# nianlonggu/WhisperSeg

Hardware: AMD Instinct MI355X
Metric: audio-sec/s segmented (whisperseg-large, 30 s windows) (higher is better)
Workload: dtype f16x3

## Files before the change

### whisperseg_amd/csrc/wseg_enc.hip

```cpp
#include <stdlib.h>
#include <string.h>
#include "wseg_kernels.h"

namespace wseg {

template <typename T>
__global__ __launch_bounds__(256) void im2col_conv1_kernel(const float* __restrict__ x, void* __restrict__ a1,
                                                           int C, int cols, int kp) {
  constexpr int TT = 32;
  __shared__ float tile[96][TT + 2 + 1];
  const int b = blockIdx.y, t0 = blockIdx.x * TT;
  for (int i = threadIdx.x; i < C * (TT + 2); i += 256) {
    const int c = i / (TT + 2), j = i - c * (TT + 2);
    const int t = t0 + j - 1;
    tile[c][j] = (t >= 0 && t < cols) ? x[((size_t)b * C + c) * cols + t] : 0.f;
  }
  __syncthreads();
  for (int i = threadIdx.x; i < TT * kp; i += 256) {
    const int tt = i / kp, k = i - tt * kp;
    if (t0 + tt >= cols) continue;
    float v = 0.f;
    if (k < 3 * C) {
      const int tap = k / C, c = k - tap * C;
      v = tile[c][tt + tap];
    }
    Op<T>::st1(a1, (size_t)b * cols + t0 + tt, kp, k, v);
  }
}

template <typename T>
__global__ __launch_bounds__(256) void im2col_conv2_kernel(const T* __restrict__ h1, T* __restrict__ a2,
                                                           int B, int cols, int d) {
  constexpr int V = 16 / sizeof(T);
  const int dv = d / V, half = cols / 2;
  const size_t total = (size_t)B * half * 3 * dv;
  for (size_t i = (size_t)blockIdx.x * 256 + threadIdx.x; i < total; i += (size_t)gridDim.x * 256) {
    const int cv = (int)(i % dv);
    const size_t r = i / dv;
    const int tap = (int)(r % 3);
    const size_t bt = r / 3;
    const int t = (int)(bt % half), b = (int)(bt / half);
    const int src = 2 * t + tap - 1;
    uint4 v = make_uint4(0, 0, 0, 0);
    if (src >= 0 && src < cols) v = *(const uint4*)(h1 + ((size_t)b * cols + src) * d + (size_t)cv * V);
    *(uint4*)(a2 + (bt * 3 + tap) * d + (size_t)cv * V) = v;
  }
}

template <typename T> struct VecIO {
  static __device__ __forceinline__ void ld(const T* p, float v[8]) { unpack8<T>(*(const uint4*)p, v); }
  static __device__ __forceinline__ void st(T* p, const float v[8]) { *(uint4*)p = pack8<T>(v); }
};
template <> struct VecIO<float> {
  static __device__ __forceinline__ void ld(const float* p, float v[8]) {
    const float4 a = *(const float4*)p, b = *(const float4*)(p + 4);
    v[0] = a.x; v[1] = a.y; v[2] = a.z; v[3] = a.w; v[4] = b.x; v[5] = b.y; v[6] = b.z; v[7] = b.w;
  }
  static __device__ __forceinline__ void st(float* p, const float v[8]) {
    *(float4*)p = make_float4(v[0], v[1], v[2], v[3]);
    *(float4*)(p + 4) = make_float4(v[4], v[5], v[6], v[7]);
  }
};

template <typename TO, int NIT>
__global__ __launch_bounds__(256) void layernorm_kernel(const float* __restrict__ x, const typename IO<TO>::P* __restrict__ g,
                                                        const typename IO<TO>::P* __restrict__ bta, void* __restrict__ y, int M, int d) {
  typedef typename IO<TO>::P PT;
  constexpr int V = 8;
  const int row = blockIdx.x * 4 + (threadIdx.x >> 6), lane = threadIdx.x & 63;
  if (row >= M) return;
  const float* xr = x + (size_t)row * d;
  float v[NIT][V];
  float sum = 0.f;
#pragma unroll
  for (int it = 0; it < NIT; ++it) {
    const int c = (it * 64 + lane) * V;
    if (c < d) {
      VecIO<float>::ld(xr + c, v[it]);
#pragma unroll
      for (int j = 0; j < V; ++j) sum += v[it][j];
    } else {
#pragma unroll
      for (int j = 0; j < V; ++j) v[it][j] = 0.f;
    }
  }
  const float mean = wave_sum(sum) / (float)d;
  float sq = 0.f;
#pragma unroll
  for (int it = 0; it < NIT; ++it) {
    const int c = (it * 64 + lane) * V;
    if (c < d) {
#pragma unroll
      for (int j = 0; j < V; ++j) { const float t = v[it][j] - mean; sq += t * t; }
    }
  }
  const float rstd = 1.0f / sqrtf(wave_sum(sq) / (float)d + 1e-5f);
#pragma unroll
  for (int it = 0; it < NIT; ++it) {
    const int c = (it * 64 + lane) * V;
    if (c < d) {
      float gg[V], bb[V], o[V];
      VecIO<PT>::ld(g + c, gg);
      VecIO<PT>::ld(bta + c, bb);
#pragma unroll
      for (int j = 0; j < V; ++j) o[j] = (v[it][j] - mean) * rstd * gg[j] + bb[j];
      op_st8<TO>(y, (size_t)row, d, c, o);
    }
  }
}

template <typename HT, typename TO, bool SPLIT = false>
__global__ __launch_bounds__(256, SPLIT ? 3 : 4) void enc_attention_h16_kernel(const HT* __restrict__ Q, const HT* __restrict__ K,
                                                                const HT* __restrict__ Vt, void* __restrict__ out,
                                                                 int H, int T, int Tp, int d, size_t plane) {
  __shared__ __attribute__((aligned(16))) HT sK[2][64 * 64];
  __shared__ __attribute__((aligned(16))) HT sV[64 * 64];
  __shared__ __attribute__((aligned(16))) HT sKl[SPLIT ? 2 : 1][SPLIT ? 64 * 64 : 8];
  __shared__ __attribute__((aligned(16))) HT sVl[SPLIT ? 64 * 64 : 8];
  const int tid = threadIdx.x, lane = tid & 63;
  const int wave = __builtin_amdgcn_readfirstlane(tid >> 6);
  const int bh = blockIdx.y, b = bh / H, h = bh - b * H;
  const int q0 = blockIdx.x * 128 + wave * 32;
  const int qi = lane & 31, g2 = lane >> 5;
  const HT* Qb = Q + enc_qk_index(bh, Tp, 0);
  const HT* Kb = K + enc_qk_index(bh, Tp, 0);
  const HT* Vb = Vt + enc_vt_block(bh, Tp);

  bf16x8 qf[4], qfl[SPLIT ? 4 : 1];
#pragma unroll
  for (int hs = 0; hs < 4; ++hs) qf[hs] = *(const bf16x8*)(Qb + (size_t)(q0 + qi) * 64 + hs * 16 + g2 * 8);
  if constexpr (SPLIT) {
#pragma unroll
    for (int hs = 0; hs < 4; ++hs) qfl[hs] = *(const bf16x8*)(Qb + plane + (size_t)(q0 + qi) * 64 + hs * 16 + g2 * 8);
  }

  f32x16 o0, o1;
#pragma unroll
  for (int r = 0; r < 16; ++r) { o0[r] = 0.f; o1[r] = 0.f; }
  float m_run = -1.0e30f, l_run = 0.f;

  const int n_tiles = (T + 63) / 64;
  const unsigned kfrag = (unsigned)(qi * 128 + ((g2 ^ ((qi >> 1) & 7)) << 4));
  constexpr int NDMA = SPLIT ? 4 : 2;
  auto fetch_tile = [&](const HT* src, HT* dst, HT* dst_lo) {
#pragma unroll
    for (int i = 0; i < 2; ++i) {
      const int c = tid + i * 256, row = c >> 3, sl = (c & 7) ^ ((row >> 1) & 7);
      __builtin_amdgcn_global_load_lds((const __attribute__((address_space(1))) void*)(src + row * 64 + sl * 8),
                                       (__attribute__((address_space(3))) void*)(dst + (i * 256 + wave * 64) * 8), 16, 0, 0);
      if constexpr (SPLIT)
        __builtin_amdgcn_global_load_lds((const __attribute__((address_space(1))) void*)(src + plane + row * 64 + sl * 8),
                                         (__attribute__((address_space(3))) void*)(dst_lo + (i * 256 + wave * 64) * 8), 16, 0, 0);
    }
  };
  auto fetch_k = [&](int kt) { fetch_tile(Kb + (size_t)(kt * 64) * 64, sK[kt & 1], sKl[kt & 1]); };
  auto fetch_v = [&](int kt) { fetch_tile(Vb + (size_t)kt * 64 * 64, sV, sVl); };
  fetch_k(0);
  for (int kt = 0; kt < n_tiles; ++kt) {
    const HT* cK = sK[kt & 1];
    asm volatile("s_waitcnt vmcnt(0)" ::: "memory");
    __syncthreads();
    fetch_v(kt);
    const bool more = kt + 1 < n_tiles;
    if (more) fetch_k(kt + 1);
    {
      const int key_base = kt * 64;
      f32x16 s0, s1;
#pragma unroll
      for (int r = 0; r < 16; ++r) { s0[r] = 0.f; s1[r] = 0.f; }
      unsigned kfo = kfrag;
      asm volatile("" : "+v"(kfo));
      const char* cKs = (const char*)cK;
      [[maybe_unused]] const char* cKls = (const char*)sKl[kt & 1];
      __builtin_amdgcn_s_setprio(1);
#pragma unroll
      for (int hs = 0; hs < 4; ++hs) {
        const bf16x8 kf0 = *(const bf16x8*)(cKs + (kfo ^ (hs << 5)));
        const bf16x8 kf1 = *(const bf16x8*)(cKs + 4096 + (kfo ^ (hs << 5)));
        s0 = H16<HT>::mfma32(kf0, qf[hs], s0);
        s1 = H16<HT>::mfma32(kf1, qf[hs], s1);
        if constexpr (SPLIT) {
          const bf16x8 kfl0 = *(const bf16x8*)(cKls + (kfo ^ (hs << 5)));
          const bf16x8 kfl1 = *(const bf16x8*)(cKls + 4096 + (kfo ^ (hs << 5)));
          s0 = H16<HT>::mfma32(kf0, qfl[hs], s0);
          s1 = H16<HT>::mfma32(kf1, qfl[hs], s1);
          s0 = H16<HT>::mfma32(kfl0, qf[hs], s0);
          s1 = H16<HT>::mfma32(kfl1, qf[hs], s1);
        }
      }
      __builtin_amdgcn_s_setprio(0);
      if (key_base + 64 > T) {
        asm volatile("");
#pragma unroll
        for (int r = 0; r < 16; ++r) {
          const int key = key_base + (r & 3) + 8 * (r >> 2) + 4 * g2;
          if (key >= T) s0[r] = -1.0e30f;
          if (key + 32 >= T) s1[r] = -1.0e30f;
        }
      }
      float mx = fmaxf(s0[0], s1[0]);
#pragma unroll
      for (int r = 1; r < 16; ++r) mx = fmaxf(fmaxf(mx, s0[r]), s1[r]);
      mx = fmaxf(mx, lane_xor<32>(mx));
      const float m_new = fmaxf(m_run, mx);
      const float alpha = __expf(m_run - m_new);
      float ps = 0.f;
      const float m_l2 = -m_new * 1.4426950408889634f;
#pragma unroll
      for (int r = 0; r < 16; ++r) {
        s0[r] = __builtin_amdgcn_exp2f(fmaf(s0[r], 1.4426950408889634f, m_l2));
        s1[r] = __builtin_amdgcn_exp2f(fmaf(s1[r], 1.4426950408889634f, m_l2));
        ps += s0[r] + s1[r];
      }
      m_run = m_new;
      if (__builtin_amdgcn_ballot_w64(alpha != 1.0f)) {
#pragma unroll
        for (int r = 0; r < 16; ++r) { o0[r] *= alpha; o1[r] *= alpha; }
      }
      if (more) asm volatile("s_waitcnt vmcnt(%0) lgkmcnt(0)" ::"n"(NDMA) : "memory");
      else asm volatile("s_waitcnt vmcnt(0) lgkmcnt(0)" ::: "memory");
      __builtin_amdgcn_s_barrier();
      asm volatile("" ::: "memory");
      __builtin_amdgcn_s_setprio(1);
#pragma unroll
      for (int sub = 0; sub < 2; ++sub) {
        const f32x16& sv = sub == 0 ? s0 : s1;
#pragma unroll
        for (int mm = 0; mm < 2; ++mm) {
          union { bf16x8 v; uint32_t u[4]; } pf, pfl;
#pragma unroll
          for (int jj = 0; jj < 4; ++jj) pf.u[jj] = H16<HT>::pack(sv[8 * mm + 2 * jj], sv[8 * mm + 2 * jj + 1]);
          if constexpr (SPLIT) {
#pragma unroll
            for (int jj = 0; jj < 4; ++jj)
              pfl.u[jj] = H16<HT>::pack(H16<HT>::sub_lo(sv[8 * mm + 2 * jj], pf.u[jj]), H16<HT>::sub_hi(sv[8 * mm + 2 * jj + 1], pf.u[jj]));
          }
#pragma unroll
          for (int ht = 0; ht < 2; ++ht) {
            const bf16x8 vf = *(const bf16x8*)((const char*)sV + ht * 4096 + (kfo ^ ((sub * 2 + mm) << 5)));
            if (ht == 0) o0 = H16<HT>::mfma32(vf, pf.v, o0);
            else o1 = H16<HT>::mfma32(vf, pf.v, o1);
            if constexpr (SPLIT) {
              const bf16x8 vfl = *(const bf16x8*)((const char*)sVl + ht * 4096 + (kfo ^ ((sub * 2 + mm) << 5)));
              if (ht == 0) { o0 = H16<HT>::mfma32(vf, pfl.v, o0); o0 = H16<HT>::mfma32(vfl, pf.v, o0); }
              else { o1 = H16<HT>::mfma32(vf, pfl.v, o1); o1 = H16<HT>::mfma32(vfl, pf.v, o1); }
            }
          }
        }
      }
      __builtin_amdgcn_s_setprio(0);
      ps += lane_xor<32>(ps);
      l_run = l_run * alpha + ps;
    }
  }
  const int q = q0 + qi;
  if constexpr (IsMx<TO>::v) {
    const float inv = 1.0f / l_run;
    uint32_t hw[2][8], lw[2][8];
    float amax_h[2] = {0.f, 0.f}, amax_l[2] = {0.f, 0.f};
#pragma unroll
    for (int ht = 0; ht < 2; ++ht) {
      const f32x16& o = ht == 0 ? o0 : o1;
#pragma unroll
      for (int p = 0; p < 8; ++p) {
        const float a0 = H16<f16_t>::sat(o[2 * p] * inv), a1 = H16<f16_t>::sat(o[2 * p + 1] * inv);
        const uint32_t hh = H16<f16_t>::pack(a0, a1);
        const float r0 = a0 - H16<f16_t>::lo(hh), r1 = a1 - H16<f16_t>::hi(hh);
        const uint32_t ll = H16<f16_t>::pack(r0, r1);
        hw[ht][p] = hh; lw[ht][p] = ll;
        amax_h[ht] = fmaxf(amax_h[ht], fmaxf(fabsf(H16<f16_t>::lo(hh)), fabsf(H16<f16_t>::hi(hh))));
        amax_l[ht] = fmaxf(amax_l[ht], fmaxf(fabsf(H16<f16_t>::lo(ll)), fabsf(H16<f16_t>::hi(ll))));
      }
    }
    uint32_t gh[16], gl[16];
    float ah = g2 ? amax_h[1] : amax_h[0], al = g2 ? amax_l[1] : amax_l[0];
    ah = fmaxf(ah, lane_xor<32>(g2 ? amax_h[0] : amax_h[1]));
    al = fmaxf(al, lane_xor<32>(g2 ? amax_l[0] : amax_l[1]));
#pragma unroll
    for (int p = 0; p < 8; ++p) {
      const uint32_t mine_h = g2 ? hw[1][p] : hw[0][p], give_h = g2 ? hw[0][p] : hw[1][p];
      const uint32_t mine_l = g2 ? lw[1][p] : lw[0][p], give_l = g2 ? lw[0][p] : lw[1][p];
      const uint32_t got_h = lane_xor_u<32>(give_h), got_l = lane_xor_u<32>(give_l);
      const int rg = p >> 1, pr = p & 1;
      gh[4 * rg + pr] = g2 ? got_h : mine_h;
      gh[4 * rg + 2 + pr] = g2 ? mine_h : got_h;
      gl[4 * rg + pr] = g2 ? got_l : mine_l;
      gl[4 * rg + 2 + pr] = g2 ? mine_l : got_l;
    }
    if (q < T) {
      const size_t row = (size_t)b * T + q;
      const int c = h * 64 + g2 * 32;
      unsigned char* blk = (unsigned char*)out + row * (size_t)(4 * d) + (size_t)(c >> 6) * 256;
#pragma unroll
      for (int i = 0; i < 4; ++i) *(uint4*)(blk + (c & 63) * 2 + 16 * i) = make_uint4(gh[4 * i], gh[4 * i + 1], gh[4 * i + 2], gh[4 * i + 3]);
      uint4 c0, c1;
      const int chunk = (c >> 5) & 1;
      mx_chunk(gl, al, c0, c1);
      *(uint4*)(blk + 128 + 32 * chunk) = c0; *(uint4*)(blk + 128 + 32 * chunk + 16) = c1;
      mx_chunk(gh, ah, c0, c1);
      *(uint4*)(blk + 128 + 32 * (2 + chunk)) = c0; *(uint4*)(blk + 128 + 32 * (2 + chunk) + 16) = c1;
    }
  } else if (q < T) {
    const float inv = 1.0f / l_run;
#pragma unroll
    for (int ht = 0; ht < 2; ++ht) {
#pragma unroll
      for (int rg = 0; rg < 4; ++rg) {
        const int hd = ht * 32 + 8 * rg + 4 * g2;
        const f32x16& o = ht == 0 ? o0 : o1;
        const float v4[4] = {o[4 * rg + 0] * inv, o[4 * rg + 1] * inv, o[4 * rg + 2] * inv, o[4 * rg + 3] * inv};
        op_st4<TO>(out, (size_t)b * T + q, d, h * 64 + hd, v4);
      }
    }
  }
}

template <typename TO>
__global__ __launch_bounds__(64) void enc_attention_f32_kernel(const float* __restrict__ Q, const float* __restrict__ K,
                                                               const float* __restrict__ Vt, void* __restrict__ out,
                                                               int H, int T, int Tp, int d) {
  const int bh = blockIdx.y, b = bh / H, h = bh - b * H;
  const int q = blockIdx.x * 64 + threadIdx.x;
  if (q >= T) return;
  const float* qp = Q + enc_qk_index(bh, Tp, q);
  float qv[64], o[64];
#pragma unroll
  for (int e = 0; e < 64; ++e) { qv[e] = qp[e]; o[e] = 0.f; }
  float mx = -3.0e38f;
  for (int t = 0; t < T; ++t) {
    const float* kp = K + enc_qk_index(bh, Tp, t);
    float s = 0.f;
#pragma unroll
    for (int e = 0; e < 64; ++e) s = fmaf(qv[e], kp[e], s);
    mx = fmaxf(mx, s);
  }
  float l = 0.f;
  for (int t = 0; t < T; ++t) {
    const float* kp = K + enc_qk_index(bh, Tp, t);
    float s = 0.f;
#pragma unroll
    for (int e = 0; e < 64; ++e) s = fmaf(qv[e], kp[e], s);
    const float p = expf(s - mx);
    l += p;
    const float* vp = Vt + vt_plain_index((size_t)bh * 64, Tp, t);
#pragma unroll
    for (int e = 0; e < 64; ++e) o[e] = fmaf(p, vp[vt_plain_index((size_t)e, Tp, 0)], o[e]);
  }
  const float inv = 1.0f / l;
#pragma unroll
  for (int e = 0; e < 64; e += 8) {
    float v8[8];
#pragma unroll
    for (int u = 0; u < 8; ++u) v8[u] = o[e + u] * inv;
    op_st8<TO>(out, (size_t)b * T + q, d, h * 64 + e, v8);
  }
}

template <typename TO>
__global__ __launch_bounds__(256) void enc_attention_f32_mfma_kernel(const float* __restrict__ Q, const float* __restrict__ K,
                                                                     const float* __restrict__ Vt, void* __restrict__ out,
                                                                     int H, int T, int Tp, int d) {
  __shared__ float sK[32][65];
  __shared__ float sV[64][33];
  __shared__ float sP[4][32][33];
  const int tid = threadIdx.x, lane = tid & 63, wave = tid >> 6, fi = lane & 31, fk = lane >> 5;
  const int bh = blockIdx.y, b = bh / H, h = bh - b * H;
  const int q0 = blockIdx.x * 128 + wave * 32;
  const float* Qb = Q + (size_t)bh * Tp * 64;
  const float* Kb = K + (size_t)bh * Tp * 64;
  const float* Vb = Vt + (size_t)bh * 64 * Tp;
  const int qrow = min(q0 + fi, Tp - 1);
  float qf[32];
#pragma unroll
  for (int kk = 0; kk < 32; ++kk) qf[kk] = Qb[(size_t)qrow * 64 + 2 * kk + fk];
  const int n_tiles = (T + 31) / 32;
  auto load_k = [&](int kt) {
#pragma unroll
    for (int i = 0; i < 2; ++i) {
      const int c = tid + i * 256, row = c >> 4, col = (c & 15) * 4;
      const float4 v = *(const float4*)(Kb + (size_t)(kt * 32 + row) * 64 + col);
      sK[row][col] = v.x; sK[row][col + 1] = v.y; sK[row][col + 2] = v.z; sK[row][col + 3] = v.w;
    }
  };
  auto load_v = [&](int kt) {
#pragma unroll
    for (int i = 0; i < 2; ++i) {
      const int c = tid + i * 256, row = c >> 3, col = (c & 7) * 4;
      const float4 v = *(const float4*)(Vb + (size_t)row * Tp + kt * 32 + col);
      sV[row][col] = v.x; sV[row][col + 1] = v.y; sV[row][col + 2] = v.z; sV[row][col + 3] = v.w;
    }
  };
  auto scores = [&](int kt, f32x16& sc) {
#pragma unroll
    for (int r = 0; r < 16; ++r) sc[r] = 0.f;
#pragma unroll
    for (int kk = 0; kk < 32; ++kk) sc = __builtin_amdgcn_mfma_f32_32x32x2f32(sK[fi][2 * kk + fk], qf[kk], sc, 0, 0, 0);
  };
  float mx = -3.0e38f;
  for (int kt = 0; kt < n_tiles; ++kt) {
    __syncthreads();
    load_k(kt);
    __syncthreads();
    f32x16 sc;
    scores(kt, sc);
#pragma unroll
    for (int r = 0; r < 16; ++r) {
      const int key = kt * 32 + 8 * (r >> 2) + 4 * fk + (r & 3);
      if (key < T) mx = fmaxf(mx, sc[r]);
    }
  }
  mx = fmaxf(mx, lane_xor<32>(mx));
  f32x16 o0, o1, la;
#pragma unroll
  for (int r = 0; r < 16; ++r) { o0[r] = 0.f; o1[r] = 0.f; la[r] = 0.f; }
  for (int kt = 0; kt < n_tiles; ++kt) {
    __syncthreads();
    load_k(kt);
    load_v(kt);
    __syncthreads();
    f32x16 sc;
    scores(kt, sc);
#pragma unroll
    for (int r = 0; r < 16; ++r) {
      const int kl = 8 * (r >> 2) + 4 * fk + (r & 3);
      sP[wave][kl][fi] = (kt * 32 + kl < T) ? expf(sc[r] - mx) : 0.f;
    }
    __builtin_amdgcn_fence(__ATOMIC_RELEASE, "wavefront");
    __builtin_amdgcn_wave_barrier();
    __builtin_amdgcn_fence(__ATOMIC_ACQUIRE, "wavefront");
#pragma unroll
    for (int kk = 0; kk < 16; ++kk) {
      const float pb = sP[wave][2 * kk + fk][fi];
      o0 = __builtin_amdgcn_mfma_f32_32x32x2f32(sV[fi][2 * kk + fk], pb, o0, 0, 0, 0);
      o1 = __builtin_amdgcn_mfma_f32_32x32x2f32(sV[32 + fi][2 * kk + fk], pb, o1, 0, 0, 0);
      la = __builtin_amdgcn_mfma_f32_32x32x2f32(1.0f, pb, la, 0, 0, 0);
    }
  }
  const int q = q0 + fi;
  if (q < T) {
    const float inv = 1.0f / la[0];
#pragma unroll
    for (int g = 0; g < 4; ++g) {
      const int hd = 8 * g + 4 * fk;
      const float a[4] = {o0[4 * g] * inv, o0[4 * g + 1] * inv, o0[4 * g + 2] * inv, o0[4 * g + 3] * inv};
      const float c[4] = {o1[4 * g] * inv, o1[4 * g + 1] * inv, o1[4 * g + 2] * inv, o1[4 * g + 3] * inv};
      op_st4<TO>(out, (size_t)b * T + q, d, h * 64 + hd, a);
      op_st4<TO>(out, (size_t)b * T + q, d, h * 64 + 32 + hd, c);
    }
  }
}

static bool is_x3(int dtype) { return dtype == WSEG_BF16X3 || dtype == WSEG_F16X3; }

template <typename HT>
__global__ __launch_bounds__(256) void operand_to_f32_kernel(const uint16_t* __restrict__ op, float* __restrict__ out, size_t n8, int d) {
  for (size_t i = (size_t)blockIdx.x * 256 + threadIdx.x; i < n8; i += (size_t)gridDim.x * 256) {
    const size_t row = i / (d >> 3);
    const int c = (int)(i - row * (d >> 3)) << 3;
    const uint16_t* p = op + row * (size_t)(2 * d) + x3_col(c);
    float h[8], l[8];
    unpack8<HT>(*(const uint4*)p, h);
    unpack8<HT>(*(const uint4*)(p + 32), l);
    float* o = out + row * d + c;
    *(float4*)o = make_float4(h[0] + l[0], h[1] + l[1], h[2] + l[2], h[3] + l[3]);
    *(float4*)(o + 4) = make_float4(h[4] + l[4], h[5] + l[5], h[6] + l[6], h[7] + l[7]);
  }
}
template <typename HT>
__global__ __launch_bounds__(256) void f32_to_operand_kernel(const float* __restrict__ in, void* __restrict__ op, size_t n8, int d) {
  for (size_t i = (size_t)blockIdx.x * 256 + threadIdx.x; i < n8; i += (size_t)gridDim.x * 256) {
    const size_t row = i / (d >> 3);
    const int c = (int)(i - row * (d >> 3)) << 3;
    float v[8];
    VecIO<float>::ld(in + row * d + c, v);
    op_st8<X3<HT>>(op, row, d, c, v);
  }
}
template <bool WORDER>
__global__ __launch_bounds__(256) void x3_to_m6_kernel(const uint16_t* __restrict__ src, unsigned char* __restrict__ dst, size_t n_groups, int K) {
  __shared__ __attribute__((aligned(16))) unsigned char stage[4][64 * 144];
  const int tid = threadIdx.x, lane = tid & 63, wave = tid >> 6;
  const int gpr = K >> 5;
  for (size_t g0 = ((size_t)blockIdx.x * 4 + wave) * 64; g0 < n_groups; g0 += (size_t)gridDim.x * 256) {
    const unsigned char* sp = (const unsigned char*)src + g0 * 128;
    const size_t n_here = n_groups - g0 < 64 ? n_groups - g0 : 64;
#pragma unroll
    for (int q = 0; q < 8; ++q) {
      const int piece = q * 64 + lane;
      const int grp = piece >> 3;
      uint4 v = make_uint4(0, 0, 0, 0);
      if ((size_t)grp < n_here) v = *(const uint4*)(sp + (size_t)piece * 16);
      *(uint4*)(stage[wave] + grp * 144 + (piece & 7) * 16) = v;
    }
    __builtin_amdgcn_fence(__ATOMIC_RELEASE, "wavefront");
    __builtin_amdgcn_wave_barrier();
    __builtin_amdgcn_fence(__ATOMIC_ACQUIRE, "wavefront");
    union { uint4 q[4]; mx_h32 h; } hi, lo;
#pragma unroll
    for (int q = 0; q < 4; ++q) { hi.q[q] = *(const uint4*)(stage[wave] + lane * 144 + q * 16); lo.q[q] = *(const uint4*)(stage[wave] + lane * 144 + 64 + q * 16); }
    __builtin_amdgcn_wave_barrier();
    if ((size_t)lane < n_here) {
      float ah = 0.f, al = 0.f;
#pragma unroll
      for (int i = 0; i < 32; ++i) { ah = fmaxf(ah, fabsf((float)hi.h[i])); al = fmaxf(al, fabsf((float)lo.h[i])); }
      const int sbh = mx_scale_byte(ah), sbl = mx_scale_byte(al);
      const mx_u6 ch = __builtin_amdgcn_cvt_scalef32_pk32_fp6_f16(hi.h, __uint_as_float((unsigned)sbh << 23));
      const mx_u6 cl = __builtin_amdgcn_cvt_scalef32_pk32_fp6_f16(lo.h, __uint_as_float((unsigned)sbl << 23));
      const size_t g = g0 + lane, row = g / gpr;
      const int gi = (int)(g - row * gpr), chunk = gi & 1;
      unsigned char* d64 = dst + row * (size_t)(4 * K) + (size_t)(gi >> 1) * 256;
#pragma unroll
      for (int q = 0; q < 4; ++q) *(uint4*)(d64 + chunk * 64 + q * 16) = hi.q[q];
      unsigned char* mx = d64 + 128;
      unsigned char* plo = mx + 32 * ((WORDER ? 2 : 0) + chunk);
      unsigned char* phi = mx + 32 * ((WORDER ? 0 : 2) + chunk);
      *(uint4*)plo = make_uint4(cl[0], cl[1], cl[2], cl[3]);
      *(uint4*)(plo + 16) = make_uint4(cl[4], cl[5], (unsigned)sbl, 0u);
      *(uint4*)phi = make_uint4(ch[0], ch[1], ch[2], ch[3]);
      *(uint4*)(phi + 16) = make_uint4(ch[4], ch[5], (unsigned)sbh, 0u);
    }
  }
}

int launch_x3_to_m6(const void* x3_rows, void* m6_rows, size_t M, int K, bool weight_order, hipStream_t s) {
  if (K <= 0 || K % 64) { set_error("x3_to_m6: K %d must be a multiple of 64", K); return WSEG_ERR_INVALID; }
  const size_t n_groups = M * (size_t)(K >> 5);
  if (n_groups == 0) return WSEG_OK;
  const size_t want = (n_groups + 255) / 256;
  const int blocks = (int)(want < 16384 ? want : 16384);
  if (weight_order) hipLaunchKernelGGL(x3_to_m6_kernel<true>, dim3(blocks), dim3(256), 0, s, (const uint16_t*)x3_rows, (unsigned char*)m6_rows, n_groups, K);
  else hipLaunchKernelGGL(x3_to_m6_kernel<false>, dim3(blocks), dim3(256), 0, s, (const uint16_t*)x3_rows, (unsigned char*)m6_rows, n_groups, K);
  WSEG_LAUNCH_CHECK();
  return WSEG_OK;
}

int launch_operand_to_f32(int dtype, const void* op, float* out, size_t M, int d, hipStream_t s) {
  if (!is_x3(dtype) || d % 32) { set_error("operand_to_f32: dtype %d / d %d unsupported", dtype, d); return WSEG_ERR_INVALID; }
  const size_t n8 = M * (size_t)(d >> 3);
  if (n8 == 0) return WSEG_OK;
  const int blocks = (int)((n8 + 255) / 256 < 16384 ? (n8 + 255) / 256 : 16384);
  if (dtype == WSEG_BF16X3) hipLaunchKernelGGL(operand_to_f32_kernel<bf16_t>, dim3(blocks), dim3(256), 0, s, (const uint16_t*)op, out, n8, d);
  else hipLaunchKernelGGL(operand_to_f32_kernel<f16_t>, dim3(blocks), dim3(256), 0, s, (const uint16_t*)op, out, n8, d);
  WSEG_LAUNCH_CHECK();
  return WSEG_OK;
}
int launch_f32_to_operand(int dtype, const float* in, void* op, size_t M, int d, hipStream_t s) {
  if (!is_x3(dtype) || d % 32) { set_error("f32_to_operand: dtype %d / d %d unsupported", dtype, d); return WSEG_ERR_INVALID; }
  const size_t n8 = M * (size_t)(d >> 3);
  if (n8 == 0) return WSEG_OK;
  const int blocks = (int)((n8 + 255) / 256 < 16384 ? (n8 + 255) / 256 : 16384);
  if (dtype == WSEG_BF16X3) hipLaunchKernelGGL(f32_to_operand_kernel<bf16_t>, dim3(blocks), dim3(256), 0, s, in, op, n8, d);
  else hipLaunchKernelGGL(f32_to_operand_kernel<f16_t>, dim3(blocks), dim3(256), 0, s, in, op, n8, d);
  WSEG_LAUNCH_CHECK();
  return WSEG_OK;
}

int launch_im2col_conv1(int dtype, const float* feats, void* a1, int B, int n_mels, int cols, int kp, hipStream_t s) {
  if (n_mels > 96 || 3 * n_mels > kp) { set_error("im2col_conv1: n_mels %d unsupported", n_mels); return WSEG_ERR_INVALID; }
  dim3 grid(cdiv(cols, 32), B);
#define WSEG_IC1(T_) hipLaunchKernelGGL((im2col_conv1_kernel<T_>), grid, dim3(256), 0, s, feats, a1, n_mels, cols, kp)
  if (dtype == WSEG_BF16) WSEG_IC1(bf16_t);
  else if (dtype == WSEG_F16) WSEG_IC1(f16_t);
  else if (dtype == WSEG_BF16X3) WSEG_IC1(X3<bf16_t>);
  else if (dtype == WSEG_F16X3) WSEG_IC1(X3<f16_t>);
  else WSEG_IC1(float);
#undef WSEG_IC1
  WSEG_LAUNCH_CHECK();
  return WSEG_OK;
}

int launch_im2col_conv2(int dtype, const void* h1, void* a2, int B, int cols, int d, hipStream_t s) {
  if (is_x3(dtype)) d *= 2;
  const size_t vec = dtype == WSEG_F32 ? 4 : 8;
  const size_t total = (size_t)B * (cols / 2) * 3 * (d / vec);
  const int blocks = (int)((total + 255) / 256 < 8192 ? (total + 255) / 256 : 8192);
  if (dtype != WSEG_F32) hipLaunchKernelGGL((im2col_conv2_kernel<bf16_t>), dim3(blocks), dim3(256), 0, s, (const bf16_t*)h1, (bf16_t*)a2, B, cols, d);
  else hipLaunchKernelGGL((im2col_conv2_kernel<float>), dim3(blocks), dim3(256), 0, s, (const float*)h1, (float*)a2, B, cols, d);
  WSEG_LAUNCH_CHECK();
  return WSEG_OK;
}

int launch_layernorm(int dtype, const float* x, const void* g, const void* b, void* y, int M, int d, hipStream_t s) {
  if (M <= 0) return WSEG_OK;
  dim3 grid(cdiv(M, 4));
  if (d % 8 || d > 64 * 8 * 4) { set_error("layernorm: d %d unsupported", d); return WSEG_ERR_INVALID; }
#define WSEG_LN(TO_, NIT_) hipLaunchKernelGGL((layernorm_kernel<TO_, NIT_>), grid, dim3(256), 0, s, x, (const typename IO<TO_>::P*)g, (const typename IO<TO_>::P*)b, y, M, d)
#define WSEG_LN3(TO_) do { if (d <= 512) WSEG_LN(TO_, 1); else if (d <= 1024) WSEG_LN(TO_, 2); else WSEG_LN(TO_, 4); } while (0)
  if (dtype == WSEG_BF16) WSEG_LN3(bf16_t);
  else if (dtype == WSEG_F16) WSEG_LN3(f16_t);
  else if (dtype == WSEG_BF16X3) WSEG_LN3(X3<bf16_t>);
  else if (dtype == WSEG_F16X3) WSEG_LN3(X3<f16_t>);
  else if (dtype == WSEG_F16M6) WSEG_LN3(M6);
  else WSEG_LN3(float);
#undef WSEG_LN3
#undef WSEG_LN
  WSEG_LAUNCH_CHECK();
  return WSEG_OK;
}

template <typename TO>
static void launch_enc_attention_f32(const void* q, const void* k, const void* vt, void* out, int B, int H, int T, int Tp, int d, hipStream_t s) {
  static const bool naive = getenv("WSEG_F32_ATTN") && !strcmp(getenv("WSEG_F32_ATTN"), "naive");
  if (naive || Tp % 128 != 0) {
    dim3 grid(cdiv(T, 64), B * H);
    hipLaunchKernelGGL(enc_attention_f32_kernel<TO>, grid, dim3(64), 0, s, (const float*)q, (const float*)k, (const float*)vt, out, H, T, Tp, d);
  } else {
    dim3 grid(cdiv(T, 128), B * H);
    hipLaunchKernelGGL(enc_attention_f32_mfma_kernel<TO>, grid, dim3(256), 0, s, (const float*)q, (const float*)k, (const float*)vt, out, H, T, Tp, d);
  }
}

bool enc_attention_writes_mx(int dtype) { return dtype == WSEG_F16M6; }
bool enc_attention_vt_tiled(int dtype) { return dtype != WSEG_F32; }

int launch_enc_attention(int dtype, const void* q, const void* k, const void* vt, void* out,
                         int B, int H, int T, int Tp, int d, hipStream_t s) {
  if (dtype == WSEG_F16M6) {
    if (Tp % 128) { set_error("enc_attention: Tp %d %% 128", Tp); return WSEG_ERR_INVALID; }
    dim3 grid(cdiv(T, 128), B * H);
    hipLaunchKernelGGL((enc_attention_h16_kernel<f16_t, M6, true>), grid, dim3(256), 0, s, (const f16_t*)q, (const f16_t*)k, (const f16_t*)vt, out, H, T, Tp, d,
                       (size_t)B * H * Tp * 64);
    WSEG_LAUNCH_CHECK();
    return WSEG_OK;
  }
  if (dtype == WSEG_BF16 || dtype == WSEG_F16 || is_x3(dtype)) {
    if (Tp % 128) { set_error("enc_attention: Tp %d %% 128", Tp); return WSEG_ERR_INVALID; }
    dim3 grid(cdiv(T, 128), B * H);
    const size_t plane = (size_t)B * H * Tp * 64;
#define WSEG_EA(HT_, TO_, SP_) hipLaunchKernelGGL((enc_attention_h16_kernel<HT_, TO_, SP_>), grid, dim3(256), 0, s, (const HT_*)q, (const HT_*)k, (const HT_*)vt, out, H, T, Tp, d, plane)
    if (dtype == WSEG_BF16) WSEG_EA(bf16_t, bf16_t, false);
    else if (dtype == WSEG_F16) WSEG_EA(f16_t, f16_t, false);
    else if (dtype == WSEG_BF16X3) WSEG_EA(f16_t, X3<bf16_t>, true);
    else WSEG_EA(f16_t, X3<f16_t>, true);
#undef WSEG_EA
  } else launch_enc_attention_f32<float>(q, k, vt, out, B, H, T, Tp, d, s);
  WSEG_LAUNCH_CHECK();
  return WSEG_OK;
}

}

extern "C" int wseg_convert_operand(const void* src_x3_rows, void* dst_m6_rows, int64_t n_rows, int32_t K, int32_t weight_order, void* stream) {
  using namespace wseg;
  if (!src_x3_rows || !dst_m6_rows || n_rows < 0 || src_x3_rows == dst_m6_rows) { set_error("wseg_convert_operand: bad argument"); return WSEG_ERR_INVALID; }
  return launch_x3_to_m6(src_x3_rows, dst_m6_rows, (size_t)n_rows, K, weight_order != 0, (hipStream_t)stream);
}
```

Baseline: 9468.

## Add dedicated split-precision encoder attention kernel with DMA-to-LDS software pipeline

Adds a separate encoder attention kernel for the x3 split-precision dtypes. It loads K/V hi and lo planes straight into swizzled LDS with buffer_load_lds, double-buffers K tiles two ahead, and interleaves the next tile's QK MFMAs with the current tile's softmax and rescale under explicit sched barriers. It also computes the P residual with v_fma_mix and uses permlane32_swap for the half-wave reductions. The aim is to hide global-load and softmax latency behind MFMA work. The cost is much more hand-scheduled code with inline asm waitcnt tuning, which is fragile to get right.

```diff
diff --git a/whisperseg_amd/csrc/wseg_enc.hip b/whisperseg_amd/csrc/wseg_enc.hip
--- a/whisperseg_amd/csrc/wseg_enc.hip
+++ b/whisperseg_amd/csrc/wseg_enc.hip
@@ -109,6 +109,31 @@
   }
 }
 
+__device__ __forceinline__ float halves_max3(float m, float v) {
+  const auto r = __builtin_amdgcn_permlane32_swap(__float_as_uint(v), __float_as_uint(v), false, false);
+  return fmaxf(m, fmaxf(__uint_as_float(r[0]), __uint_as_float(r[1])));
+}
+__device__ __forceinline__ float halves_sum(float v) {
+  const auto r = __builtin_amdgcn_permlane32_swap(__float_as_uint(v), __float_as_uint(v), false, false);
+  return __uint_as_float(r[0]) + __uint_as_float(r[1]);
+}
+template <typename HT> struct PResid {
+  static __device__ __forceinline__ float lo(float s, uint32_t w) { return H16<HT>::sub_lo(s, w); }
+  static __device__ __forceinline__ float hi(float s, uint32_t w) { return H16<HT>::sub_hi(s, w); }
+};
+template <> struct PResid<f16_t> {
+  static __device__ __forceinline__ float lo(float s, uint32_t w) {
+    float r;
+    asm("v_fma_mix_f32 %0, %1, -1.0, %2 op_sel_hi:[1,0,0]" : "=v"(r) : "v"(w), "v"(s));
+    return r;
+  }
+  static __device__ __forceinline__ float hi(float s, uint32_t w) {
+    float r;
+    asm("v_fma_mix_f32 %0, %1, -1.0, %2 op_sel:[1,0,0] op_sel_hi:[1,0,0]" : "=v"(r) : "v"(w), "v"(s));
+    return r;
+  }
+};
+
 template <typename HT, typename TO, bool SPLIT = false>
 __global__ __launch_bounds__(256, SPLIT ? 3 : 4) void enc_attention_h16_kernel(const HT* __restrict__ Q, const HT* __restrict__ K,
                                                                 const HT* __restrict__ Vt, void* __restrict__ out,
@@ -315,6 +340,227 @@
   }
 }
 
+template <typename HT, typename TO>
+__global__ __launch_bounds__(256, 3) void enc_attention_x3_kernel(const HT* __restrict__ Q, const HT* __restrict__ K, const HT* __restrict__ Vt,
+                                                                  void* __restrict__ out, int H, int T, int Tp, int d, size_t plane) {
+  __shared__ __attribute__((aligned(16))) HT sK0[64 * 64], sK1[64 * 64], sKl0[64 * 64], sKl1[64 * 64];
+  __shared__ __attribute__((aligned(16))) HT sV[64 * 64], sVl[64 * 64];
+  const int tid = threadIdx.x, lane = tid & 63;
+  const int wave = __builtin_amdgcn_readfirstlane(tid >> 6);
+  const int bh = blockIdx.y, b = bh / H, h = bh - b * H;
+  const int q0 = blockIdx.x * 128 + wave * 32;
+  const int qi = lane & 31, g2 = lane >> 5;
+  const HT* Qb = Q + enc_qk_index(bh, Tp, 0);
+  const HT* Kb = K + enc_qk_index(bh, Tp, 0);
+  const HT* Vb = Vt + enc_vt_block(bh, Tp);
+
+  bf16x8 qf[4], qfl[4];
+#pragma unroll
+  for (int hs = 0; hs < 4; ++hs) {
+    qf[hs] = *(const bf16x8*)(Qb + (size_t)(q0 + qi) * 64 + hs * 16 + g2 * 8);
+    qfl[hs] = *(const bf16x8*)(Qb + plane + (size_t)(q0 + qi) * 64 + hs * 16 + g2 * 8);
+  }
+  f32x16 o0, o1;
+#pragma unroll
+  for (int r = 0; r < 16; ++r) { o0[r] = 0.f; o1[r] = 0.f; }
+  float m_run = -1.0e30f, l_run = 0.f;
+  const int n_tiles = (T + 63) / 64;
+  const unsigned kfrag = (unsigned)(qi * 128 + ((g2 ^ ((qi >> 1) & 7)) << 4));
+  constexpr int NDMA = 4;
+  const unsigned foff = (unsigned)(((tid >> 3) * 64 + (((tid & 7) ^ ((tid >> 4) & 7)) << 3)) * sizeof(HT));
+  auto block_rsrc = [&](const HT* p) { return __builtin_amdgcn_make_buffer_rsrc((void*)p, 0, Tp * 64 * (int)sizeof(HT), 0x00020000); };
+  const __amdgpu_buffer_rsrc_t rK = block_rsrc(Kb), rKl = block_rsrc(Kb + plane), rV = block_rsrc(Vb), rVl = block_rsrc(Vb + plane);
+  auto fetch_tile = [&](const __amdgpu_buffer_rsrc_t& src, const __amdgpu_buffer_rsrc_t& src_lo, int kt, HT* dst, HT* dst_lo) {
+#pragma unroll
+    for (int i = 0; i < 2; ++i) {
+      const int so = (kt * 4096 + i * 2048) * (int)sizeof(HT);
+      __builtin_amdgcn_raw_ptr_buffer_load_lds(src, (__attribute__((address_space(3))) void*)(dst + (i * 256 + wave * 64) * 8), 16, foff, so, 0, 0);
+      __builtin_amdgcn_raw_ptr_buffer_load_lds(src_lo, (__attribute__((address_space(3))) void*)(dst_lo + (i * 256 + wave * 64) * 8), 16, foff, so, 0, 0);
+    }
+  };
+  auto fetch_k = [&](auto par_c, int kt) {
+    if constexpr (decltype(par_c)::value == 0) fetch_tile(rK, rKl, kt, sK0, sKl0);
+    else fetch_tile(rK, rKl, kt, sK1, sKl1);
+  };
+  auto fetch_v = [&](int kt) { fetch_tile(rV, rVl, kt, sV, sVl); };
+  auto scores = [&](const HT* cK, const HT* cKl, unsigned kfo, f32x16& a0, f32x16& a1) {
+#pragma unroll
+    for (int r = 0; r < 16; ++r) { a0[r] = 0.f; a1[r] = 0.f; }
+    const char* cKs = (const char*)cK;
+    const char* cKls = (const char*)cKl;
+#pragma unroll
+    for (int hs = 0; hs < 4; ++hs) {
+      const bf16x8 kf0 = *(const bf16x8*)(cKs + (kfo ^ (hs << 5)));
+      const bf16x8 kf1 = *(const bf16x8*)(cKs + 4096 + (kfo ^ (hs << 5)));
+      const bf16x8 kfl0 = *(const bf16x8*)(cKls + (kfo ^ (hs << 5)));
+      const bf16x8 kfl1 = *(const bf16x8*)(cKls + 4096 + (kfo ^ (hs << 5)));
+      a0 = H16<HT>::mfma32(kf0, qf[hs], a0);
+      a1 = H16<HT>::mfma32(kf1, qf[hs], a1);
+      a0 = H16<HT>::mfma32(kf0, qfl[hs], a0);
+      a1 = H16<HT>::mfma32(kf1, qfl[hs], a1);
+      a0 = H16<HT>::mfma32(kfl0, qf[hs], a0);
+      a1 = H16<HT>::mfma32(kfl1, qf[hs], a1);
+    }
+  };
+  auto step = [&](auto last_c, auto par_c, int kt, f32x16& s0, f32x16& s1, f32x16& n0, f32x16& n1) {
+    constexpr bool LAST = decltype(last_c)::value;
+    constexpr int PAR = decltype(par_c)::value;
+    asm volatile("s_waitcnt vmcnt(0)" ::: "memory");
+    __syncthreads();
+    fetch_v(kt);
+    if constexpr (!LAST) fetch_k(par_c, kt + 2);
+    unsigned kfo = kfrag;
+    asm volatile("" : "+v"(kfo));
+    float alpha, ps = 0.f;
+    if constexpr (!LAST) {
+      const char* cKs = (const char*)(PAR ? sK0 : sK1);
+      const char* cKls = (const char*)(PAR ? sKl0 : sKl1);
+      auto rd = [&](const char* base, int hs, int half) { return *(const bf16x8*)(base + half * 4096 + (kfo ^ (hs << 5))); };
+      bf16x8 kf[2], kfl[2];
+      kf[0] = rd(cKs, 0, 0);
+      kf[1] = rd(cKs, 0, 1);
+#pragma unroll
+      for (int r = 0; r < 16; ++r) { n0[r] = 0.f; n1[r] = 0.f; }
+      float mx = 0.f, m_l2 = 0.f;
+      auto rescale = [&](int i) { if (i < 16) o0[i] *= alpha; else o1[i - 16] *= alpha; };
+#pragma unroll
+      for (int g = 0; g < 24; ++g) {
+        const int hs = g / 6, pr = (g % 6) >> 1, half = g & 1;
+        __builtin_amdgcn_sched_barrier(0);
+        f32x16& acc = half ? n1 : n0;
+        if (pr == 0) {
+          if (!half) { kfl[0] = rd(cKls, hs, 0); kfl[1] = rd(cKls, hs, 1); }
+          acc = H16<HT>::mfma32(kf[half], qf[hs], acc);
+        } else if (pr == 1) {
+          acc = H16<HT>::mfma32(kf[half], qfl[hs], acc);
+        } else {
+          acc = H16<HT>::mfma32(kfl[half], qf[hs], acc);
+          if (half && hs < 3) { kf[0] = rd(cKs, hs + 1, 0); kf[1] = rd(cKs, hs + 1, 1); }
+        }
+        if (g < 4) {
+          if (g == 0) mx = fmaxf(s0[0], s1[0]);
+#pragma unroll
+          for (int r = (g == 0 ? 1 : 4 * g); r < 4 * g + 4; ++r) mx = fmaxf(fmaxf(mx, s0[r]), s1[r]);
+          asm volatile("" : "+v"(mx));
+        } else if (g == 4) {
+          const float m_new = halves_max3(m_run, mx);
+          alpha = __expf(m_run - m_new);
+          m_l2 = -m_new * 1.4426950408889634f;
+          m_run = m_new;
+          asm volatile("" : "+v"(alpha), "+v"(m_l2));
+        } else if (g >= 6 && g < 22) {
+          const int r = g - 6;
+          s0[r] = __builtin_amdgcn_exp2f(fmaf(s0[r], 1.4426950408889634f, m_l2));
+          s1[r] = __builtin_amdgcn_exp2f(fmaf(s1[r], 1.4426950408889634f, m_l2));
+          ps = r == 0 ? s0[r] + s1[r] : ps + (s0[r] + s1[r]);
+          rescale(r);
+          asm volatile("" : "+v"(ps));
+        } else if (g >= 22) {
+#pragma unroll
+          for (int i = 0; i < 8; ++i) rescale(16 + 8 * (g - 22) + i);
+        }
+      }
+      __builtin_amdgcn_sched_barrier(0);
+    } else {
+      const int key_base = kt * 64;
+      if (key_base + 64 > T) {
+        int tl = tid;
+        asm volatile("" : "+v"(tl));
+        const int g2l = (tl >> 5) & 1;
+#pragma unroll
+        for (int r = 0; r < 16; ++r) {
+          const int key = key_base + (r & 3) + 8 * (r >> 2) + 4 * g2l;
+          if (key >= T) s0[r] = -1.0e30f;
+          if (key + 32 >= T) s1[r] = -1.0e30f;
+        }
+      }
+      float mx = fmaxf(s0[0], s1[0]);
+#pragma unroll
+      for (int r = 1; r < 16; ++r) mx = fmaxf(fmaxf(mx, s0[r]), s1[r]);
+      const float m_new = halves_max3(m_run, mx);
+      alpha = __expf(m_run - m_new);
+      const float m_l2 = -m_new * 1.4426950408889634f;
+#pragma unroll
+      for (int r = 0; r < 16; ++r) {
+        s0[r] = __builtin_amdgcn_exp2f(fmaf(s0[r], 1.4426950408889634f, m_l2));
+        s1[r] = __builtin_amdgcn_exp2f(fmaf(s1[r], 1.4426950408889634f, m_l2));
+        ps = r == 0 ? s0[r] + s1[r] : ps + (s0[r] + s1[r]);
+      }
+      m_run = m_new;
+      if (__builtin_amdgcn_ballot_w64(alpha != 1.0f)) {
+#pragma unroll
+        for (int r = 0; r < 16; ++r) { o0[r] *= alpha; o1[r] *= alpha; }
+      }
+    }
+    if constexpr (!LAST) asm volatile("s_waitcnt vmcnt(%0) lgkmcnt(0)" ::"n"(NDMA) : "memory");
+    else asm volatile("s_waitcnt vmcnt(0) lgkmcnt(0)" ::: "memory");
+    __builtin_amdgcn_s_barrier();
+    asm volatile("" ::: "memory");
+#pragma unroll
+    for (int G = 0; G < 4; ++G) {
+      const f32x16& sv = G < 2 ? s0 : s1;
+      const int mm = G & 1;
+      union { bf16x8 v; uint32_t u[4]; } pf, pfl;
+#pragma unroll
+      for (int jj = 0; jj < 4; ++jj) pf.u[jj] = H16<HT>::pack(sv[8 * mm + 2 * jj], sv[8 * mm + 2 * jj + 1]);
+#pragma unroll
+      for (int jj = 0; jj < 4; ++jj)
+        pfl.u[jj] = H16<HT>::pack(PResid<HT>::lo(sv[8 * mm + 2 * jj], pf.u[jj]), PResid<HT>::hi(sv[8 * mm + 2 * jj + 1], pf.u[jj]));
+#pragma unroll
+      for (int ht = 0; ht < 2; ++ht) {
+        const bf16x8 vf = *(const bf16x8*)((const char*)sV + ht * 4096 + (kfo ^ (G << 5)));
+        const bf16x8 vfl = *(const bf16x8*)((const char*)sVl + ht * 4096 + (kfo ^ (G << 5)));
+        if (ht == 0) { o0 = H16<HT>::mfma32(vf, pf.v, o0); o0 = H16<HT>::mfma32(vf, pfl.v, o0); o0 = H16<HT>::mfma32(vfl, pf.v, o0); }
+        else { o1 = H16<HT>::mfma32(vf, pf.v, o1); o1 = H16<HT>::mfma32(vf, pfl.v, o1); o1 = H16<HT>::mfma32(vfl, pf.v, o1); }
+      }
+    }
+    l_run = l_run * alpha + halves_sum(ps);
+  };
+
+  using P0 = std::integral_constant<int, 0>;
+  using P1 = std::integral_constant<int, 1>;
+  fetch_k(P0{}, 0);
+  if (n_tiles > 1) {
+    fetch_k(P1{}, 1);
+    asm volatile("s_waitcnt vmcnt(%0)" ::"n"(NDMA) : "memory");
+  } else {
+    asm volatile("s_waitcnt vmcnt(0)" ::: "memory");
+  }
+  __builtin_amdgcn_s_barrier();
+  asm volatile("" ::: "memory");
+  f32x16 a0, a1, b0, b1;
+  scores(sK0, sKl0, kfrag, a0, a1);
+  int kt = 0;
+  for (; kt + 2 < n_tiles; kt += 2) {
+    step(std::false_type{}, P0{}, kt, a0, a1, b0, b1);
+    step(std::false_type{}, P1{}, kt + 1, b0, b1, a0, a1);
+  }
+  if (kt + 1 < n_tiles) {
+    step(std::false_type{}, P0{}, kt, a0, a1, b0, b1);
+    a0 = b0;
+    a1 = b1;
+    ++kt;
+  }
+  step(std::true_type{}, P0{}, kt, a0, a1, b0, b1);
+
+  int te = tid;
+  asm volatile("" : "+v"(te));
+  const int q = blockIdx.x * 128 + (te >> 6) * 32 + (te & 31), g2e = (te >> 5) & 1;
+  if (q < T) {
+    const float inv = 1.0f / l_run;
+#pragma unroll
+    for (int ht = 0; ht < 2; ++ht) {
+#pragma unroll
+      for (int rg = 0; rg < 4; ++rg) {
+        const int hd = ht * 32 + 8 * rg + 4 * g2e;
+        const f32x16& o = ht == 0 ? o0 : o1;
+        const float v4[4] = {o[4 * rg + 0] * inv, o[4 * rg + 1] * inv, o[4 * rg + 2] * inv, o[4 * rg + 3] * inv};
+        op_st4<TO>(out, (size_t)b * T + q, d, h * 64 + hd, v4);
+      }
+    }
+  }
+}
+
 template <typename TO>
 __global__ __launch_bounds__(64) void enc_attention_f32_kernel(const float* __restrict__ Q, const float* __restrict__ K,
                                                                const float* __restrict__ Vt, void* __restrict__ out,
@@ -627,11 +873,14 @@
     if (Tp % 128) { set_error("enc_attention: Tp %d %% 128", Tp); return WSEG_ERR_INVALID; }
     dim3 grid(cdiv(T, 128), B * H);
     const size_t plane = (size_t)B * H * Tp * 64;
+#define WSEG_EAX(TO_) hipLaunchKernelGGL((enc_attention_x3_kernel<f16_t, TO_>), grid, dim3(256), 0, s, (const f16_t*)q, (const f16_t*)k, (const f16_t*)vt, out, H, T, Tp, d, plane)
 #define WSEG_EA(HT_, TO_, SP_) hipLaunchKernelGGL((enc_attention_h16_kernel<HT_, TO_, SP_>), grid, dim3(256), 0, s, (const HT_*)q, (const HT_*)k, (const HT_*)vt, out, H, T, Tp, d, plane)
     if (dtype == WSEG_BF16) WSEG_EA(bf16_t, bf16_t, false);
     else if (dtype == WSEG_F16) WSEG_EA(f16_t, f16_t, false);
-    else if (dtype == WSEG_BF16X3) WSEG_EA(f16_t, X3<bf16_t>, true);
-    else WSEG_EA(f16_t, X3<f16_t>, true);
+    else if (T < 1) { set_error("enc_attention: T %d", T); return WSEG_ERR_INVALID; }
+    else if (dtype == WSEG_BF16X3) WSEG_EAX(X3<bf16_t>);
+    else WSEG_EAX(X3<f16_t>);
+#undef WSEG_EAX
 #undef WSEG_EA
   } else launch_enc_attention_f32<float>(q, k, vt, out, B, H, T, Tp, d, s);
   WSEG_LAUNCH_CHECK();
```

Measured after the change: 9478 (median of 5 runs). About the same (+0.1%).
